# G-U-N/a-PyTorch-Tutorial-to-Class-Incremental-Learning

Measured on AMD Instinct MI355X. Metric: imgs/sec/node (CIFAR-100 B0-Inc10 ResNet-18 WA+KD step), higher is better.
Workload: dtype bf16; 1 GPU; model=resnet18, global_batch=128, input_size=32, kd=True, hip_graph=True, parallelism=dp1

## Files before the change

### cilfw/_hip_ops.py

```python

import ctypes
import os

import torch

_LIB_PATH = os.path.join(os.path.dirname(os.path.abspath(__file__)),
                         "_hip_lib.so")
if not os.path.exists(_LIB_PATH):
    raise ImportError(f"cilfw HIP library not built: {_LIB_PATH}")
_lib = ctypes.CDLL(_LIB_PATH)

_DEBUG = os.environ.get("CILFW_SYNC_DEBUG") == "1"

c_vp = ctypes.c_void_p
c_i = ctypes.c_int
c_l = ctypes.c_long
c_f = ctypes.c_float

_lib.cilfw_sync.restype = c_i
_lib.cilfw_error_string.restype = ctypes.c_char_p
_lib.cilfw_error_string.argtypes = [c_i]

_PROTOS = {
    "cilfw_conv2d_fwd": [c_vp] * 4 + [c_i] * 12 + [c_vp, c_vp],
    "cilfw_conv2d_bwd_data": [c_vp] * 4 + [c_i] * 12 + [c_vp] * 5 + [c_i, c_vp],
    "cilfw_conv2d_bwd_weight": [c_vp] * 4 + [c_i] * 13 + [c_vp],
    "cilfw_fill_mtable": [c_vp] + [c_i] * 4 + [c_vp],
    "cilfw_im2col_smallc": [c_vp] * 3 + [c_i] * 11 + [c_vp],
    "cilfw_bn_apply_only": [c_vp] * 7 + [c_l, c_i, c_i, c_vp],
    "cilfw_bn_fwd": [c_vp] * 11 + [c_i, c_l, c_i, c_f, c_f, c_i, c_i, c_vp],
    "cilfw_bn_bwd": [c_vp] * 11 + [c_vp, c_i] + [c_l, c_i, c_i, c_i, c_vp],
    "cilfw_add_relu_fwd": [c_vp] * 3 + [c_l, c_vp],
    "cilfw_add_relu_bwd": [c_vp] * 3 + [c_l, c_vp],
    "cilfw_downsample_a_fwd": [c_vp] * 2 + [c_i] * 4 + [c_vp],
    "cilfw_downsample_a_bwd": [c_vp] * 2 + [c_i] * 4 + [c_vp],
    "cilfw_gap_fwd": [c_vp] * 2 + [c_i] * 3 + [c_vp],
    "cilfw_gap_bwd": [c_vp] * 2 + [c_i] * 3 + [c_vp],
    "cilfw_stride_gather": [c_vp] * 2 + [c_i] * 7 + [c_vp],
    "cilfw_stride_scatter": [c_vp] * 2 + [c_i] * 7 + [c_vp],
    "cilfw_maxpool_fwd": [c_vp] * 3 + [c_i] * 9 + [c_vp],
    "cilfw_maxpool_bwd": [c_vp] * 3 + [c_i] * 9 + [c_vp],
    "cilfw_linear_fwd": [c_vp] * 5 + [c_i] * 4 + [c_vp],
    "cilfw_linear_dx": [c_vp] * 4 + [c_i] * 4 + [c_vp],
    "cilfw_linear_dw": [c_vp] * 5 + [c_i] * 4 + [c_vp],
    "cilfw_ce_fwd": [c_vp] * 5 + [c_i, c_i, c_f, c_vp],
    "cilfw_ce_bwd": [c_vp] * 4 + [c_i, c_i, c_f, c_vp],
    "cilfw_kd_fwd": [c_vp] * 6 + [c_i, c_i, c_f, c_vp],
    "cilfw_kd_bwd": [c_vp] * 4 + [c_i, c_i, c_f, c_vp],
    "cilfw_wa_loss_fwd": [c_vp] * 8 + [c_i] * 3 + [c_f] * 3 + [c_vp],
    "cilfw_wa_loss_bwd": [c_vp] * 6 + [c_i] * 3 + [c_f] * 3 + [c_vp],
    "cilfw_sgd_step": [c_vp] * 4 + [c_l, c_vp, c_f, c_f, c_vp],
    "cilfw_topk_correct": [c_vp] * 3 + [c_i] * 3 + [c_vp],
    "cilfw_herding_select": [c_vp] * 3 + [c_i] * 3 + [c_vp],
    "cilfw_herding_select_batch": [c_vp] * 6 + [c_i] * 3 + [c_vp],
    "cilfw_crop_resize": [c_vp] * 7 + [c_i] * 7 + [c_vp],
    "cilfw_crop_resize_ragged": [c_vp] * 9 + [c_i] * 5 + [c_vp],
    "cilfw_nme_prototypes": [c_vp] * 3 + [c_i] * 2 + [c_vp],
    "cilfw_nme_topk": [c_vp] * 6 + [c_i] * 4 + [c_vp],
    "cilfw_pod_pool": [c_vp] * 2 + [c_i] * 4 + [c_vp],
    "cilfw_pod_dist": [c_vp] * 5 + [c_i] * 2 + [c_vp],
    "cilfw_pod_bwd": [c_vp] * 4 + [c_i] * 4 + [c_vp],
    "cilfw_rownorm_fwd": [c_vp] * 4 + [c_i] * 3 + [c_vp],
    "cilfw_rownorm_bwd": [c_vp] * 6 + [c_i] * 3 + [c_vp],
    "cilfw_cos_sum": [c_vp] * 2 + [c_i, c_f, c_vp],
    "cilfw_flat_dist": [c_vp] * 5 + [c_i] * 2 + [c_vp],
    "cilfw_flat_bwd": [c_vp] * 3 + [c_i] * 2 + [c_vp],
    "cilfw_mrank_fwd": [c_vp] * 9 + [c_i] * 4 + [c_f, c_vp],
    "cilfw_mrank_bwd": [c_vp] * 6 + [c_i] * 4 + [c_vp],
}
for _name, _args in _PROTOS.items():
    _fn = getattr(_lib, _name)
    _fn.argtypes = _args
    _fn.restype = None

_lib.cilfw_conv2d_bwd_data.restype = c_i
for _name in ("cilfw_pod_pool", "cilfw_pod_dist", "cilfw_pod_bwd",
              "cilfw_rownorm_fwd", "cilfw_rownorm_bwd", "cilfw_cos_sum",
              "cilfw_flat_dist", "cilfw_flat_bwd", "cilfw_mrank_fwd",
              "cilfw_mrank_bwd"):
    getattr(_lib, _name).restype = c_i

for _name, _n in [("cilfw_linear_ksplit", 3),
                  ("cilfw_conv2d_fwd_ksplit", 7),
                  ("cilfw_conv2d_bwd_data_ksplit", 7),
                  ("cilfw_conv2d_bwd_data_can_fuse_bn", 8),
                  ("cilfw_conv2d_bwd_data_bn_gy", 3),
                  ("cilfw_conv2d_fwd_bn_gy", 3),
                  ("cilfw_bnbwd_fuse_enabled", 0),
                  ("cilfw_conv2d_bwd_weight_nslices", 7),
                  ("cilfw_conv2d_fwd_route", 8),
                  ("cilfw_conv2d_bwd_data_route", 9),
                  ("cilfw_conv2d_bwd_weight_route", 8),
                  ("cilfw_pod_supported", 4),
                  ("cilfw_pod_pool_groups", 2),
                  ("cilfw_cosine_supported", 3),
                  ("cilfw_mrank_supported", 4)]:
    _fn = getattr(_lib, _name)
    _fn.argtypes = [c_i] * _n
    _fn.restype = c_i
_lib.cilfw_bn_sums_gy.argtypes = [c_l]
_lib.cilfw_bn_sums_gy.restype = c_i

_FWD_ROUTES = ("v1_bk32", "v1_bk64", "v2_bn64", "v2_bn128")
_BWD_DATA_ROUTES = ("s2_fused", "v2", "v1_bk32", "v1_bk64")
_BWD_WEIGHT_ROUTES = ("v2", "v1_fast", "v1_generic")


def _stream():
    return c_vp(torch.cuda.current_stream().cuda_stream)


def _ptr(t):
    return c_vp(0 if t is None else t.data_ptr())


def _check(name):
    if _DEBUG:
        e = _lib.cilfw_sync()
        if e != 0:
            raise RuntimeError(
                f"HIP error after {name}: "
                f"{_lib.cilfw_error_string(e).decode()}")


def _bf16(t, name):
    assert t.dtype == torch.bfloat16, \
        f"{name}: GPU compute path is bf16 (got {t.dtype}); run with " \
        f"--dtype bf16 or set CILFW_FORCE_TORCH=1 for debugging"
    assert t.is_contiguous(), f"{name}: needs contiguous tensor"
    return t



def _out_hw(H, W_, R, S, stride, pad):
    return ((H + 2 * pad - R) // stride + 1,
            (W_ + 2 * pad - S) // stride + 1)


def _crs_pad(C, R, S):
    return (C * R * S + 15) // 16 * 16


def _slab_ws(nslabs, numel, device, always=False):
    if nslabs > 1 or always:
        return torch.empty(nslabs * numel, dtype=torch.float32, device=device)
    return None


def _stem_as_1x1(x, R, S, stride, pad, Ho, Wo):
    N, H, W_, C = x.shape
    M, CRSpad = N * Ho * Wo, _crs_pad(C, R, S)
    mt = _mtable(N, Ho, Wo, stride, x.device)
    col = torch.zeros(M, 1, 1, CRSpad, dtype=torch.bfloat16, device=x.device)
    _lib.cilfw_im2col_smallc(_ptr(x), _ptr(mt), _ptr(col), c_i(N), c_i(H),
                             c_i(W_), c_i(C), c_i(R), c_i(S), c_i(stride),
                             c_i(pad), c_i(Ho), c_i(Wo), c_i(CRSpad),
                             _stream())
    _check("im2col_smallc")
    return col


def conv2d_fwd_route(N, H, W_, C, K, R, S, stride, pad):
    Ho, Wo = _out_hw(H, W_, R, S, stride, pad)
    ks = _lib.cilfw_conv2d_fwd_ksplit(N, C, K, R, S, Ho, Wo)
    return _FWD_ROUTES[_lib.cilfw_conv2d_fwd_route(N, C, K, R, S, Ho, Wo,
                                                   ks)], ks


def conv2d_bwd_data_route(N, H, W_, C, K, R, S, stride):
    if R == 1 and S == 1 and stride > 1:
        H, W_, stride = (H - 1) // stride + 1, (W_ - 1) // stride + 1, 1
    ks = _lib.cilfw_conv2d_bwd_data_ksplit(N, H, W_, C, K, R, S)
    return _BWD_DATA_ROUTES[_lib.cilfw_conv2d_bwd_data_route(
        N, H, W_, C, K, R, S, stride, ks)], ks


def bnbwd_fuse_enabled():
    return bool(_lib.cilfw_bnbwd_fuse_enabled())


def _stem_im2col_dw(C, K, R, S):
    use_im2col = (os.environ.get("CILFW_STEM_IM2COL") == "1"
                  or (R * S >= 25
                      and os.environ.get("CILFW_STEM_IM2COL") != "0"))
    return C < 16 and R * S > 1 and K % 16 == 0 and use_im2col


def conv2d_bwd_weight_route(N, C, K, R, S, Ho, Wo, accum=False):
    if _stem_im2col_dw(C, K, R, S):
        N, C, R, S, Ho, Wo = N * Ho * Wo, _crs_pad(C, R, S), 1, 1, 1, 1
        accum = False
    ns = _lib.cilfw_conv2d_bwd_weight_nslices(N, C, K, R, S, Ho, Wo)
    return _BWD_WEIGHT_ROUTES[_lib.cilfw_conv2d_bwd_weight_route(
        N, C, K, R, S, Ho, Wo, 1 if accum else 0)], ns


def conv2d_fwd(x, w, stride, pad, want_bn_parts=False):
    _bf16(x, "conv2d_fwd.x")
    _bf16(w, "conv2d_fwd.w")
    N, H, W_, C = x.shape
    R, S, Cw, K = w.shape
    assert Cw == C
    assert K % 8 == 0, "conv kernels vector-stage over output channels (K%8==0)"
    Ho, Wo = _out_hw(H, W_, R, S, stride, pad)
    if C < 16 and R * S > 1 and K % 16 == 0 \
            and os.environ.get("CILFW_STEM_IM2COL") == "1":
        col = _stem_as_1x1(x, R, S, stride, pad, Ho, Wo)
        wpad = torch.zeros(1, 1, col.shape[-1], K, dtype=torch.bfloat16,
                           device=x.device)
        wpad[0, 0, :C * R * S] = w.reshape(C * R * S, K)
        y, _ = conv2d_fwd(col, wpad, 1, 0)
        return y.view(N, Ho, Wo, K), None
    y = torch.empty(N, Ho, Wo, K, dtype=torch.bfloat16, device=x.device)
    ks = _lib.cilfw_conv2d_fwd_ksplit(N, C, K, R, S, Ho, Wo)
    ws = _slab_ws(ks, y.numel(), x.device)
    parts = None
    if want_bn_parts and ks == 1 \
            and _FWD_ROUTES[_lib.cilfw_conv2d_fwd_route(
                N, C, K, R, S, Ho, Wo, ks)].startswith("v2_") \
            and os.environ.get("CILFW_CONV_BN_FUSE", "1") != "0":
        parts = torch.empty(_lib.cilfw_conv2d_fwd_bn_gy(N, Ho, Wo), 2, K,
                            dtype=torch.float32, device=x.device)
    _lib.cilfw_conv2d_fwd(_ptr(x), _ptr(w), _ptr(y), _ptr(ws), c_i(N),
                          c_i(H), c_i(W_), c_i(C), c_i(K), c_i(R), c_i(S),
                          c_i(stride), c_i(pad), c_i(Ho), c_i(Wo), c_i(ks),
                          _ptr(parts), _stream())
    _check("conv2d_fwd")
    return y, parts


def conv2d_bwd_data(dy, w, stride, pad, H, W_, bn_meta=None):
    _bf16(dy, "conv2d_bwd_data.dy")
    N, Ho, Wo, K = dy.shape
    R, S, C, Kw = w.shape
    assert Kw == K
    if R == 1 and S == 1 and stride > 1:
        dxs = conv2d_bwd_data(dy, w, 1, 0, Ho, Wo)
        dx = torch.empty(N, H, W_, C, dtype=torch.bfloat16, device=dy.device)
        _lib.cilfw_stride_scatter(_ptr(dxs), _ptr(dx), c_i(N), c_i(H),
                                  c_i(W_), c_i(C), c_i(stride), c_i(Ho),
                                  c_i(Wo), _stream())
        _check("stride_scatter")
        return (dx, None) if bn_meta is not None else dx
    dx = torch.empty(N, H, W_, C, dtype=torch.bfloat16, device=dy.device)
    ks = _lib.cilfw_conv2d_bwd_data_ksplit(N, H, W_, C, K, R, S)
    ws = _slab_ws(ks, dx.numel(), dy.device)
    parts = None
    bn_y = bn_x = bn_mean = bn_invstd = None
    bn_relu = False
    if (bn_meta is not None
            and _lib.cilfw_conv2d_bwd_data_can_fuse_bn(
                N, H, W_, C, K, R, S, stride)):
        bn_y, bn_x, bn_mean, bn_invstd, bn_relu = bn_meta
        parts = torch.empty(_lib.cilfw_conv2d_bwd_data_bn_gy(N, H, W_), 2, C,
                            dtype=torch.float32, device=dy.device)
    fused = _lib.cilfw_conv2d_bwd_data(
        _ptr(dy), _ptr(w), _ptr(dx), _ptr(ws), c_i(N), c_i(H), c_i(W_),
        c_i(C), c_i(K), c_i(R), c_i(S), c_i(stride), c_i(pad), c_i(Ho),
        c_i(Wo), c_i(ks), _ptr(bn_y), _ptr(bn_x), _ptr(bn_mean),
        _ptr(bn_invstd), _ptr(parts), c_i(1 if bn_relu else 0), _stream())
    if not fused:
        parts = None
    _check("conv2d_bwd_data")
    if bn_meta is not None:
        return dx, parts
    return dx


_mtable_cache = {}


def _mtable(N, Ho, Wo, stride, device):
    key = (N, Ho, Wo, stride, device)
    mt = _mtable_cache.get(key)
    if mt is None:
        assert N < 4096 and Ho * stride < 1024 and Wo * stride < 1024, \
            "mtable packing limits exceeded"
        M = N * Ho * Wo
        mt = torch.empty(M, dtype=torch.int32, device=device)
        _lib.cilfw_fill_mtable(_ptr(mt), c_i(M), c_i(Ho * Wo), c_i(Wo),
                               c_i(stride), _stream())
        _mtable_cache[key] = mt
    return mt


def conv2d_bwd_weight(dy, x, stride, pad, R, S, out=None, accum=False):
    _bf16(dy, "conv2d_bwd_weight.dy")
    _bf16(x, "conv2d_bwd_weight.x")
    N, H, W_, C = x.shape
    _, Ho, Wo, K = dy.shape
    if _stem_im2col_dw(C, K, R, S):
        col = _stem_as_1x1(x, R, S, stride, pad, Ho, Wo)
        dwp = conv2d_bwd_weight(dy.view(-1, 1, 1, K), col, 1, 0, 1, 1)
        dw = dwp.view(-1, K)[:C * R * S].reshape(R, S, C, K)
        if out is None:
            return dw
        (out.add_(dw) if accum else out.copy_(dw))
        return out
    if R == 1 and S == 1 and stride > 1:
        xg = torch.empty(N, Ho, Wo, C, dtype=torch.bfloat16, device=x.device)
        _lib.cilfw_stride_gather(_ptr(x), _ptr(xg), c_i(N), c_i(H), c_i(W_),
                                 c_i(C), c_i(stride), c_i(Ho), c_i(Wo),
                                 _stream())
        _check("stride_gather")
        return conv2d_bwd_weight(dy, xg, 1, 0, R, S, out=out, accum=accum)
    if out is None:
        dw = torch.empty(R, S, C, K, dtype=torch.float32, device=dy.device)
        accum = False
    else:
        assert out.is_contiguous() and out.dtype == torch.float32 \
            and out.shape == (R, S, C, K)
        dw = out
    ns = _lib.cilfw_conv2d_bwd_weight_nslices(N, C, K, R, S, Ho, Wo)
    ws = _slab_ws(ns, dw.numel(), dy.device, always=True)
    _lib.cilfw_conv2d_bwd_weight(_ptr(dy), _ptr(x), _ptr(dw),
                                 _ptr(ws), c_i(N), c_i(H), c_i(W_), c_i(C),
                                 c_i(K), c_i(R), c_i(S), c_i(stride),
                                 c_i(pad), c_i(Ho), c_i(Wo), c_i(ns),
                                 c_i(1 if accum else 0), _stream())
    _check("conv2d_bwd_weight")
    return dw



def bn_fwd(x, gamma, beta, running_mean, running_var, momentum, eps, training,
# ... 768 lines not shown
```

### cilfw/csrc/conv.hip

```cpp

#include "common.h"

#define BM 128
#define BN 64
#define NTHREADS 256

struct ConvGeom {
  int N, H, W, C, K, R, S, stride, pad, pad2, Ho, Wo;
  unsigned long long m_howo, m_wo;
  unsigned long long m_ck, m_s;
};

static inline unsigned long long magic40(int d) {
  return d > 0 ? ((1ULL << 40) / (unsigned)d + 1) : 0;
}

DEV unsigned mdiv40(unsigned n, unsigned long long m) {
  return (unsigned)(((unsigned long long)n * m) >> 40);
}

__global__ __launch_bounds__(NTHREADS)
void reduce_slabs_bf16_kernel(const float* __restrict__ ws,
                              bf16_t* __restrict__ out, int ns, long len) {
  long i0 = ((long)blockIdx.x * NTHREADS + threadIdx.x) * 4;
// ... 1278 lines not shown
      bool bok = m_ok & (ko0 + wv * 16 + lh * 8 + 8 <= g.K);
      const bf16_t* srcB = bok
          ? &dy[(long)mcl * g.K + ko0 + wv * 16 + lh * 8]
          : zpage;
      __builtin_amdgcn_global_load_lds(
          (const __attribute__((address_space(1))) unsigned int*)srcB,
          (__attribute__((address_space(3))) unsigned int*)
              &base[W2_IMG + wv * (WBK * 16) + i * 32 * 16], 16, 0, 0);
    }
  };

  const int fh = lane & 15, fq = lane >> 4;
  const unsigned lds0 = (unsigned)(uintptr_t)&lds[0];
  const unsigned tr_e = (unsigned)((fq * 8 + ((lane >> 2) & 3)) * 16
                                   + (lane & 3) * 4);

  const int nk = cdiv_i(me - ms, WBK);
  if (nk > 0) stage(0, ms);
  asm volatile("s_waitcnt vmcnt(0)" ::: "memory");
  __builtin_amdgcn_s_barrier();
  for (int kt = 0; kt < nk; ++kt) {
    int cur = kt & 1;
    if (kt + 1 < nk) stage(cur ^ 1, ms + (kt + 1) * WBK);
    const unsigned abase = lds0 + 2u * (cur * 2 * W2_IMG);
    const unsigned bbase = abase + 2u * W2_IMG;
    typedef __attribute__((ext_vector_type(4))) short s4_t;
#pragma unroll
    for (int kh = 0; kh < 2; ++kh) {
      const unsigned khe = 2u * (tr_e + kh * 32 * 16);
      bf16x8 afr[2], bfr[2];
#pragma unroll
      for (int mr = 0; mr < 2; ++mr) {
        unsigned a = abase + 2u * ((wr * 2 + mr) * (WBK * 16)) + khe;
        s4_t lo, hi;
        asm volatile("ds_read_b64_tr_b16 %0, %2\n\t"
                     "ds_read_b64_tr_b16 %1, %2 offset:128\n\t"
                     : "=&v"(lo), "=&v"(hi) : "v"(a));
        afr[mr] = __builtin_shufflevector(lo, hi, 0, 1, 2, 3, 4, 5, 6, 7);
      }
#pragma unroll
      for (int nr = 0; nr < 2; ++nr) {
        unsigned a = bbase + 2u * ((wc * 2 + nr) * (WBK * 16)) + khe;
        s4_t lo, hi;
        asm volatile("ds_read_b64_tr_b16 %0, %2\n\t"
                     "ds_read_b64_tr_b16 %1, %2 offset:128\n\t"
                     : "=&v"(lo), "=&v"(hi) : "v"(a));
        bfr[nr] = __builtin_shufflevector(lo, hi, 0, 1, 2, 3, 4, 5, 6, 7);
      }
      if (kh == 0) {
        asm volatile("s_waitcnt lgkmcnt(0)" ::: "memory");
        __builtin_amdgcn_sched_barrier(0);
        __builtin_amdgcn_s_setprio(1);
      } else {
        asm volatile("s_waitcnt lgkmcnt(0)" ::: "memory");
        __builtin_amdgcn_sched_barrier(0);
      }
#pragma unroll
      for (int mr = 0; mr < 2; ++mr)
#pragma unroll
        for (int nr = 0; nr < 2; ++nr)
          acc[mr][nr] = __builtin_amdgcn_mfma_f32_16x16x32_bf16(
              afr[mr], bfr[nr], acc[mr][nr], 0, 0, 0);
    }
    __builtin_amdgcn_s_setprio(0);
    asm volatile("s_waitcnt vmcnt(0)" ::: "memory");
    __builtin_amdgcn_s_barrier();
  }

  const long slab = (long)blockIdx.z * CRS * g.K;
#pragma unroll
  for (int mr = 0; mr < 2; ++mr)
#pragma unroll
    for (int nr = 0; nr < 2; ++nr)
#pragma unroll
      for (int r = 0; r < 4; ++r) {
        int row = rs0 + wr * 32 + mr * 16 + fq * 4 + r;
        int col = ko0 + wc * 32 + nr * 16 + fh;
        if (row < CRS && col < g.K)
          ws[slab + (long)row * g.K + col] = acc[mr][nr][r];
      }
}


#include <stdio.h>

#define KNOB_NEVER (1 << 30)

static int bk64_min_crs() {
  static const int v = env_int("CILFW_CONV_BK64_MIN", 512);
  return v > 0 ? v : KNOB_NEVER;
}

static int bk64_max_blocks() {
  static const int v = env_int("CILFW_CONV_BK64_MAXBLOCKS", 768);
  return v;
}

static int ksplit_target() {
  static const int v = env_int("CILFW_CONV_KSPLIT_TARGET", 512);
  return v;
}

static int dw_target() {
  static const int v = env_int("CILFW_CONV_DW_TARGET", 1024);
  return v;
}

static int conv_v2_enabled() {
  static const int v = env_int("CILFW_CONV_V2", 1);
  return v;
}

static int conv_v2_bwd_minm() {
  static const int v = env_int("CILFW_CONV_V2_BWD_MINM", 150000);
  return v == 0 ? KNOB_NEVER : v;
}

static int fwd_bm256_min_m() {
  static const int v = env_int("CILFW_CONV_BM256_MIN", 0);
  return v > 0 ? v : KNOB_NEVER;
}

static int v2_bn128_enabled() {
  static const int v = env_int("CILFW_CONV_V2_BN128", 1);
  return v;
}

static int v2_bn128_min3x3() {
  static const int v = env_int("CILFW_CONV_V2_BN128_MIN3X3", -1);
  return v >= 0 ? v : KNOB_NEVER;
}

static int s2_fused_enabled() {
  static const int v = !env_set("CILFW_NO_S2_FUSED");
  return v;
}

static int bnbwd_fuse_enabled() {
  static const int v = env_int("CILFW_BNBWD_FUSE", 0);
  return v;
}

static int pick_ksplit(int nblocks, int nk) {
  int ks = 1;
  while (ks < 8 && nblocks * ks < ksplit_target() && nk / (ks * 2) >= 4)
    ks *= 2;
  return ks;
}

static dim3 reduce_slabs_grid(long len) {
  return dim3((unsigned)((len + NTHREADS * 4 - 1) / (NTHREADS * 4)));
}

static void launch_reduce_slabs_bf16(const void* ws, void* out, int ksplit,
                                     long len, void* stream) {
  if (ksplit <= 1) return;
  hipLaunchKernelGGL(reduce_slabs_bf16_kernel, reduce_slabs_grid(len),
                     dim3(NTHREADS), 0, (hipStream_t)stream,
                     (const float*)ws, (bf16_t*)out, ksplit, len);
}

static void launch_reduce_slabs_f32(const void* ws, void* out, int nslices,
                                    long len, int accum, void* stream) {
  hipLaunchKernelGGL(reduce_slabs_f32_kernel, reduce_slabs_grid(len),
                     dim3(NTHREADS), 0, (hipStream_t)stream,
                     (const float*)ws, (float*)out, nslices, len, accum);
}

typedef void (*FwdV1Kernel)(const bf16_t*, const bf16_t*, bf16_t*, float*,
                            ConvGeom, int, int, int, int);
static const FwdV1Kernel kFwdV1[3][2] = {
    {conv2d_fwd_kernel<32, 128, BN, false>,
     conv2d_fwd_kernel<32, 128, BN, true>},
    {conv2d_fwd_kernel<64, 128, BN, false>,
     conv2d_fwd_kernel<64, 128, BN, true>},
    {conv2d_fwd_kernel<32, 256, BN, false>,
     conv2d_fwd_kernel<32, 256, BN, true>}};

typedef void (*BwdDataKernel)(const bf16_t*, const bf16_t*, bf16_t*, float*,
                              ConvGeom, int, int, int, int, const bf16_t*,
                              const bf16_t*, const float*, const float*,
                              float*, int);
static const BwdDataKernel kBwdData[2][2][2] = {
    {{conv2d_bwd_data_kernel<32, false, false>,
      conv2d_bwd_data_kernel<32, false, true>},
     {conv2d_bwd_data_kernel<32, true, false>,
      conv2d_bwd_data_kernel<32, true, true>}},
    {{conv2d_bwd_data_kernel<64, false, false>,
      conv2d_bwd_data_kernel<64, false, true>},
     {conv2d_bwd_data_kernel<64, true, false>,
      conv2d_bwd_data_kernel<64, true, true>}}};

extern "C" {

static void* zpage_ptr() {
  static void* p = nullptr;
  if (p == nullptr) {
    hipStreamCaptureStatus st = hipStreamCaptureStatusNone;
    (void)hipStreamIsCapturing(nullptr, &st);
    if (st != hipStreamCaptureStatusNone) return nullptr;
    void* q = nullptr;
    if (hipMalloc(&q, 65536) != hipSuccess) return nullptr;
    (void)hipMemset(q, 0, 65536);
    p = q;
  }
  return p;
}

enum { FWD_V1_BK32 = 0, FWD_V1_BK64 = 1, FWD_V2_BN64 = 2, FWD_V2_BN128 = 3 };
enum { BWDD_S2_FUSED = 0, BWDD_V2 = 1, BWDD_V1_BK32 = 2, BWDD_V1_BK64 = 3 };
enum { BWDW_V2 = 0, BWDW_V1_FAST = 1, BWDW_V1_GENERIC = 2 };

static int fwd_bm(int M) { return (M >= fwd_bm256_min_m()) ? 256 : BM; }

static int fwd_v2_eligible(int C) { return C % 8 == 0 && conv_v2_enabled(); }

static int fwd_route(int M, int C, int K, int R, int S, int ksplit,
                     int have_zp) {
  int CRS = C * R * S;
  int bm = fwd_bm(M);
  if (have_zp && fwd_v2_eligible(C) && bm == BM) {
    int shape_ok = (R == 1 && S == 1) || M >= v2_bn128_min3x3();
// ... 61 lines not shown
}

static int bwd_data_route(int N, int H, int W, int C, int K, int R, int S,
                          int stride, int ksplit, int have_zp) {
  int H2max = (H + 1) >> 1, W2max = (W + 1) >> 1;
  int Mc = N * H2max * W2max;
  if (stride == 2 && (R > 1 || S > 1) && K % 16 == 0 &&
      cdiv(Mc, BM) * cdiv(C, BN) >= 128 && s2_fused_enabled())
    return BWDD_S2_FUSED;
  int M = N * H * W;
  if (have_zp && bwd_data_v2_eligible(M, K, stride)) return BWDD_V2;
  int use64 = (R * S * K >= bk64_min_crs()) &&
              (cdiv(M, BM) * cdiv(C, BN) * ksplit < bk64_max_blocks());
  return use64 ? BWDD_V1_BK64 : BWDD_V1_BK32;
}

int cilfw_conv2d_bwd_data_route(int N, int H, int W, int C, int K, int R,
                                int S, int stride, int ksplit) {
  return bwd_data_route(N, H, W, C, K, R, S, stride, ksplit, 1);
}

int cilfw_conv2d_bwd_data_ksplit(int N, int H, int W, int C, int K, int R,
                                 int S) {
  return pick_ksplit(cdiv(N * H * W, BM) * cdiv(C, BN), cdiv(R * S * K, 32));
}

int cilfw_conv2d_bwd_data_can_fuse_bn(int N, int H, int W, int C, int K,
                                      int R, int S, int stride) {
  if (!bnbwd_fuse_enabled() || stride != 1) return 0;
  int ks = cilfw_conv2d_bwd_data_ksplit(N, H, W, C, K, R, S);
  int route = bwd_data_route(N, H, W, C, K, R, S, stride, ks, 1);
  return (route == BWDD_V1_BK32 || route == BWDD_V1_BK64) && ks == 1;
}

int cilfw_conv2d_bwd_data_bn_gy(int N, int H, int W) {
  return cdiv(N * H * W, BM);
}

int cilfw_conv2d_bwd_data(const void* dy, const void* w, void* dx, void* ws,
                          int N, int H, int W, int C, int K, int R, int S,
                          int stride, int pad, int Ho, int Wo, int ksplit,
                          const void* bn_y, const void* bn_x,
                          const void* bn_mean, const void* bn_invstd,
                          void* bn_parts, int bn_relu, void* stream) {
  ConvGeom g{N, H, W, C, K, R, S, stride, pad, pad, Ho, Wo,
             0, 0, magic40(K), magic40(S)};
  int M = N * H * W;
  int RSK = R * S * K;
  void* zp = bwd_data_v2_eligible(M, K, stride) ? zpage_ptr() : nullptr;
  int route = bwd_data_route(N, H, W, C, K, R, S, stride, ksplit,
                             zp != nullptr);
  if (route == BWDD_S2_FUSED) {
    int Mc = N * ((H + 1) >> 1) * ((W + 1) >> 1);
    dim3 grid(cdiv(Mc, BM), cdiv(C, BN), 4);
    hipLaunchKernelGGL((conv2d_bwd_data_s2_kernel<32>), grid, dim3(NTHREADS),
                       0, (hipStream_t)stream, (const bf16_t*)dy,
                       (const bf16_t*)w, (bf16_t*)dx, g);
    return 0;
  }
  dim3 grid(cdiv(M, BM), cdiv(C, BN), ksplit);
  int bnp = 0;
  if (route == BWDD_V2) {
    hipLaunchKernelGGL(conv2d_bwd_data_v2_kernel, grid, dim3(NTHREADS), 0,
                       (hipStream_t)stream, (const bf16_t*)dy,
                       (const bf16_t*)w, (bf16_t*)dx, (float*)ws,
                       (const bf16_t*)zp, g, M, RSK, cdiv(RSK, V2BK), ksplit);
  } else {
    int bk64 = route == BWDD_V1_BK64;
    int fast = (K % 16 == 0) && stride <= 2;
    bnp = bn_parts != nullptr && ksplit == 1 && stride == 1 &&
          bnbwd_fuse_enabled();
    hipLaunchKernelGGL(kBwdData[bk64][fast][bnp], grid, dim3(NTHREADS), 0,
                       (hipStream_t)stream, (const bf16_t*)dy,
                       (const bf16_t*)w, (bf16_t*)dx, (float*)ws, g, M, RSK,
                       cdiv(RSK, bk64 ? 64 : 32), ksplit,
                       (const bf16_t*)bn_y, (const bf16_t*)bn_x,
                       (const float*)bn_mean, (const float*)bn_invstd,
                       (float*)bn_parts, bn_relu);
  }
  launch_reduce_slabs_bf16(ws, dx, ksplit, (long)M * C, stream);
  return bnp;
}

static int bwd_weight_v2_eligible(int C, int K, int accum) {
  return C % 8 == 0 && K % 8 == 0 && accum == 0 && conv_v2_enabled();
}

static int bwd_weight_route(int C, int K, int accum, int have_zp) {
  if (have_zp && bwd_weight_v2_eligible(C, K, accum)) return BWDW_V2;
  return (C % 8 == 0) ? BWDW_V1_FAST : BWDW_V1_GENERIC;
}

int cilfw_conv2d_bwd_weight_route(int N, int C, int K, int R, int S, int Ho,
                                  int Wo, int accum) {
  (void)N; (void)R; (void)S; (void)Ho; (void)Wo;
  return bwd_weight_route(C, K, accum, 1);
}

void cilfw_conv2d_bwd_weight(const void* dy, const void* x, void* dw,
                             void* ws, int N, int H, int W, int C, int K,
                             int R, int S, int stride, int pad, int Ho,
                             int Wo, int nslices, int accum, void* stream) {
  ConvGeom g{N, H, W, C, K, R, S, stride, pad, pad, Ho, Wo,
             magic40(Ho * Wo), magic40(Wo), magic40(C), magic40(S)};
  int M = N * Ho * Wo;
  if (M >= (1 << 22) || Ho * Wo >= (1 << 14)) {
    fprintf(stderr, "cilfw_conv2d_bwd_weight: magic-division range exceeded "
            "(M=%d HoWo=%d)\n", M, Ho * Wo);
    abort();
  }
  int CRS = C * R * S;
  int slice_len = cdiv(cdiv(M, nslices), WBK) * WBK;
  dim3 grid(cdiv(CRS, WBM), cdiv(K, BN), nslices);
  void* zp = bwd_weight_v2_eligible(C, K, accum) ? zpage_ptr() : nullptr;
  int route = bwd_weight_route(C, K, accum, zp != nullptr);
  if (route == BWDW_V2)
    hipLaunchKernelGGL(conv2d_bwd_weight_v2_kernel, grid, dim3(NTHREADS), 0,
                       (hipStream_t)stream, (const bf16_t*)dy,
                       (const bf16_t*)x, (float*)ws, (const bf16_t*)zp, g,
                       M, CRS, slice_len);
  else
    hipLaunchKernelGGL(route == BWDW_V1_FAST
                           ? conv2d_bwd_weight_kernel<true>
                           : conv2d_bwd_weight_kernel<false>,
                       grid, dim3(NTHREADS), 0, (hipStream_t)stream,
                       (const bf16_t*)dy, (const bf16_t*)x, (float*)ws, g, M,
                       CRS, slice_len);
  launch_reduce_slabs_f32(ws, dw, nslices, (long)CRS * K, accum, stream);
}

void cilfw_im2col_smallc(const void* x, const void* mt, void* col,
                         int N, int H, int W, int C, int R, int S,
                         int stride, int pad, int Ho, int Wo, int CRSpad,
                         void* stream) {
  ConvGeom g{N, H, W, C, 0, R, S, stride, pad, pad, Ho, Wo};
  int M = N * Ho * Wo;
  long total = (long)M * R * S;
  hipLaunchKernelGGL(im2col_smallc_kernel,
                     dim3((int)cdiv((long)total, (long)NTHREADS)),
                     dim3(NTHREADS), 0, (hipStream_t)stream,
                     (const bf16_t*)x, (const int*)mt, (bf16_t*)col, g, M,
                     CRSpad, total);
}

void cilfw_fill_mtable(void* mt, int M, int HoWo, int Wo, int stride,
                       void* stream) {
  hipLaunchKernelGGL(fill_mtable_kernel, dim3(cdiv(M, NTHREADS)),
                     dim3(NTHREADS), 0, (hipStream_t)stream, (int*)mt, M,
                     HoWo, Wo, stride);
}

int cilfw_conv2d_bwd_weight_nslices(int N, int C, int K, int R, int S,
                                    int Ho, int Wo) {
  int M = N * Ho * Wo;
  int CRS = C * R * S;
  int nblocks = cdiv(CRS, WBM) * cdiv(K, BN);
  int ns = cdiv(dw_target(), max(nblocks, 1));
  int max_ns = max(cdiv(M, WBK * 8), 1);
  if (ns > max_ns) ns = max_ns;
  if (ns < 1) ns = 1;
  if (ns > 64) ns = 64;
  return ns;
}

}
```

### cilfw/distributed/ddp.py

```python

import torch
import torch.distributed as dist


def _dist_active():
    return dist.is_available() and dist.is_initialized() and \
        dist.get_world_size() > 1


class DataParallelEngine:
    def __init__(self, model, bucket_mb=25.0, process_group=None):
        self.model = model
        self.group = process_group
        self.params = [p for p in model.parameters() if p.requires_grad]
        self.params = self.params[::-1]
        assert all(p.dtype == torch.float32 for p in self.params), \
            "cilfw keeps fp32 master params; compute casts are per-op"
        dev = self.params[0].device
        self.numel = sum(p.numel() for p in self.params)
        self.flat_params = torch.empty(self.numel, dtype=torch.float32, device=dev)
        self.flat_grads = torch.zeros(self.numel, dtype=torch.float32, device=dev)

        offset = 0
        self._offsets = []
        for p in self.params:
            n = p.numel()
            self.flat_params[offset:offset + n].copy_(p.data.reshape(-1))
            p.data = self.flat_params[offset:offset + n].view_as(p)
            p.grad = self.flat_grads[offset:offset + n].view_as(p)
            self._offsets.append(offset)
            offset += n

        bucket_elems = max(int(bucket_mb * 1024 * 1024 / 4), 1)
        self.buckets = []
        start, count, idxs = 0, 0, []
        for i, p in enumerate(self.params):
            idxs.append(i)
            count += p.numel()
            if count >= bucket_elems:
                self.buckets.append((start, start + count, tuple(idxs)))
                start += count
                count, idxs = 0, []
        if idxs:
            self.buckets.append((start, start + count, tuple(idxs)))
        self._param_bucket = {}
        for bi, (_, _, idxs) in enumerate(self.buckets):
            for i in idxs:
                self._param_bucket[i] = bi

        self._arrived = [0] * len(self.buckets)
        self._launched = [False] * len(self.buckets)
        self._works = []
        self._hooks = []
        self._hook_enabled = True
        for i, p in enumerate(self.params):
            self._hooks.append(p.register_post_accumulate_grad_hook(
                self._make_hook(i)))

        self._epoch = 0
        self._side_dirty = False
        for i, p in enumerate(self.params):
            p._cilfw_sink = (self, i)
            p._cilfw_sink_epoch = -1

        if _dist_active():
            dist.broadcast(self.flat_params, src=0, group=self.group)

        self.flat_bf16 = None
        if self.flat_params.is_cuda:
            self.flat_bf16 = self.flat_params.to(torch.bfloat16)
            for p, off in zip(self.params, self._offsets):
                p._cilfw_bf16 = self.flat_bf16[off:off + p.numel()].view_as(p)

    def _make_hook(self, i):
        bi = self._param_bucket[i]

        def hook(_p):
            if not self._hook_enabled:
                return
            self._arrived[bi] += 1
            if self._arrived[bi] == len(self.buckets[bi][2]):
                self._launch(bi)
        return hook

    def _launch(self, bi):
        if self._launched[bi] or not _dist_active():
            self._launched[bi] = True
            return
        self._join_side_stream()
        s, e, _ = self.buckets[bi]
        work = dist.all_reduce(self.flat_grads[s:e], op=dist.ReduceOp.SUM,
                               group=self.group, async_op=True)
        self._works.append(work)
        self._launched[bi] = True


    def sink_acquire(self, i):
        p = self.params[i]
        off = self._offsets[i]
        view = self.flat_grads[off:off + p.numel()]
        return view, p._cilfw_sink_epoch == self._epoch

    def sink_delivered(self, i, side_stream=False):
        p = self.params[i]
        p._cilfw_sink_epoch = self._epoch
        if side_stream:
            self._side_dirty = True
        if self._hook_enabled:
            bi = self._param_bucket[i]
            self._arrived[bi] += 1
            if self._arrived[bi] == len(self.buckets[bi][2]):
                self._launch(bi)

    def _join_side_stream(self):
        if self._side_dirty and self.flat_grads.is_cuda:
            from ..ops.functional import _wstream
            torch.cuda.current_stream().wait_stream(_wstream())
        self._side_dirty = False

    def zero_grad(self):
        self.flat_grads.zero_()
        self._arrived = [0] * len(self.buckets)
        self._launched = [False] * len(self.buckets)
        self._works = []
        self._epoch += 1

    def finalize(self):
        for bi in range(len(self.buckets)):
            if not self._launched[bi]:
                self._launch(bi)
        self._join_side_stream()
        for w in self._works:
            w.wait()
        self._works = []
        if _dist_active():
            self.flat_grads.mul_(1.0 / dist.get_world_size(group=self.group))

    def no_sync(self):
        engine = self

        class _NoSync:
            def __enter__(self):
                engine._hook_enabled = False

            def __exit__(self, *a):
                engine._hook_enabled = True
        return _NoSync()

    def detach(self):
        for h in self._hooks:
            h.remove()
        for p in self.params:
            p.data = p.data.clone()
            p.grad = None
            if hasattr(p, "_cilfw_bf16"):
                del p._cilfw_bf16
            if hasattr(p, "_cilfw_sink"):
                del p._cilfw_sink
                del p._cilfw_sink_epoch
```

### cilfw/ops/functional.py

```python

import torch
import torch.nn.functional as F

from ._backend import use_hip, ext, _load


_wgrad_stream = None


def _wstream():
    global _wgrad_stream
    if _wgrad_stream is None:
        _wgrad_stream = torch.cuda.Stream()
    return _wgrad_stream


def _to_nchw(x):
    return x.permute(0, 3, 1, 2).contiguous()


def _to_nhwc(x):
    return x.permute(0, 2, 3, 1).contiguous()




def _sink_on():
    import os
    return os.environ.get("CILFW_SINK_MODE", "join") != "off"


def _bnbwd_fuse_on():
    E = _load()
    if E is not None:
        return E.bnbwd_fuse_enabled()
    import os
    return os.environ.get("CILFW_BNBWD_FUSE", "0") == "1"


def _conv_bwd_data_with_bn(ctx, E, dy, wc, stride, padding, x):
    meta = getattr(ctx, "bnbwd_src", None)
    if meta is None or not _bnbwd_fuse_on():
        return E.conv2d_bwd_data(dy, wc, stride, padding,
                                 x.shape[1], x.shape[2])
    bn_x, bn_mean, bn_invstd, bn_relu = meta
    dx, parts = E.conv2d_bwd_data(
        dy, wc, stride, padding, x.shape[1], x.shape[2],
        bn_meta=(x, bn_x, bn_mean, bn_invstd, bn_relu))
    if parts is not None:
        dx._cilfw_bnbwd = (parts, bn_mean)
    return dx


class Conv2dNHWC(torch.autograd.Function):

    @staticmethod
    def forward(ctx, x, w, stride, padding, w_param=None):
        ctx.stride, ctx.padding = stride, padding
        if w_param is not None:
            w_param = w_param[0]
        wp = w_param if w_param is not None else w
        wc = getattr(wp, "_cilfw_bf16", None)
        if wc is None or wc.dtype != x.dtype:
            wc = w.to(x.dtype)
        ctx.save_for_backward(x, wc)
        ctx.w_dtype = w.dtype
        ctx.w_ref = wp
        ctx.sinked = w_param is not None
        ctx.bnbwd_src = getattr(x, "_cilfw_bnbwd_src", None)
        if use_hip(x):
            y, parts = ext().conv2d_fwd(x, wc, stride, padding,
                                        want_bn_parts=ctx.sinked)
            if parts is not None:
                y._cilfw_bn_parts = parts
            return y
        xf = _to_nchw(x).float()
        wf = w.permute(3, 2, 0, 1).contiguous().float()
        y = F.conv2d(xf, wf, stride=stride, padding=padding)
        return _to_nhwc(y).to(x.dtype)

    @staticmethod
    def backward(ctx, dy):
        x, wc = ctx.saved_tensors
        stride, padding = ctx.stride, ctx.padding
        dy = dy.contiguous()
        need_dx = ctx.needs_input_grad[0]
        sink = getattr(ctx.w_ref, "_cilfw_sink", None) if ctx.sinked else None
        if use_hip(dy):
            R, S = wc.shape[0], wc.shape[1]
            cur = torch.cuda.current_stream()
            ws = _wstream()
            ws.wait_stream(cur)
            if sink is not None:
                eng, pi = sink
                slot, accum = eng.sink_acquire(pi)
                out = slot.view(R, S, wc.shape[2], wc.shape[3])
                with torch.cuda.stream(ws):
                    ext().conv2d_bwd_weight(dy, x, stride, padding, R, S,
                                            out=out, accum=accum)
                dx = _conv_bwd_data_with_bn(ctx, ext(), dy, wc, stride, padding, x) \
                    if need_dx else None
                cur.wait_stream(ws)
                eng.sink_delivered(pi)
                return dx, None, None, None, None
            with torch.cuda.stream(ws):
                dw = ext().conv2d_bwd_weight(dy, x, stride, padding, R, S)
            dx = _conv_bwd_data_with_bn(ctx, ext(), dy, wc, stride, padding, x) \
                if need_dx else None
            cur.wait_stream(ws)
            dw.record_stream(cur)
            return dx, dw.to(ctx.w_dtype), None, None, None
        xf = _to_nchw(x).float()
        wf = wc.permute(3, 2, 0, 1).contiguous().float()
        dyf = _to_nchw(dy).float()
        dx = None
        if need_dx:
            dxf = torch.nn.grad.conv2d_input(xf.shape, wf, dyf, stride=stride,
                                             padding=padding)
            dx = _to_nhwc(dxf).to(x.dtype)
        dwf = torch.nn.grad.conv2d_weight(xf, wf.shape, dyf, stride=stride,
                                          padding=padding)
        dw = dwf.permute(2, 3, 1, 0).contiguous().to(ctx.w_dtype)
        if sink is not None:
            eng, pi = sink
            slot, accum = eng.sink_acquire(pi)
            out = slot.view_as(dw)
            (out.add_(dw) if accum else out.copy_(dw))
# ... 630 lines not shown
```

### cilfw/optim.py

```python

import math

import torch

from .ops._backend import use_hip, ext


class FlatSGD:
    def __init__(self, engine, lr, momentum=0.9, weight_decay=5e-4):
        self.engine = engine
        self._lr_dev = (torch.full((1,), float(lr), dtype=torch.float32,
                                   device=engine.flat_params.device)
                        if engine.flat_params.is_cuda else None)
        self._lr = float(lr)
        self.base_lr = lr
        self.momentum = momentum
        self.weight_decay = weight_decay
        self.momentum_buf = torch.zeros_like(engine.flat_grads)

    @property
    def lr(self):
        return self._lr

    @lr.setter
    def lr(self, v):
        self._lr = float(v)
        if self._lr_dev is not None:
            self._lr_dev.fill_(float(v))

    @torch.no_grad()
    def step(self):
        p, g, m = (self.engine.flat_params, self.engine.flat_grads,
                   self.momentum_buf)
        mirror = getattr(self.engine, "flat_bf16", None)
        if use_hip(p):
            ext().sgd_step(p, g, m, self._lr_dev, self.momentum,
                           self.weight_decay, mirror)
            return
        if self.weight_decay != 0:
            g = g.add(p, alpha=self.weight_decay)
        m.mul_(self.momentum).add_(g)
        p.add_(m, alpha=-self.lr)
        if mirror is not None:
            mirror.copy_(p)

    def zero_grad(self):
        self.engine.zero_grad()

    def state_dict(self):
        return {"lr": self.lr, "base_lr": self.base_lr,
                "momentum": self.momentum, "weight_decay": self.weight_decay,
                "momentum_buf": self.momentum_buf}

    def load_state_dict(self, sd):
        self.lr = sd["lr"]
        self.base_lr = sd["base_lr"]
        self.momentum = sd["momentum"]
        self.weight_decay = sd["weight_decay"]
        self.momentum_buf.copy_(sd["momentum_buf"])


class CosineLR:

    def __init__(self, optimizer, t_max, eta_min=0.0):
        self.opt = optimizer
        self.t_max = t_max
        self.eta_min = eta_min
        self.epoch = 0

    def step(self):
        self.epoch += 1
        self.opt.lr = self.eta_min + (self.opt.base_lr - self.eta_min) * \
            (1 + math.cos(math.pi * min(self.epoch, self.t_max) / self.t_max)) / 2

    def state_dict(self):
        return {"epoch": self.epoch, "t_max": self.t_max, "eta_min": self.eta_min}

    def load_state_dict(self, sd):
        self.epoch = sd["epoch"]
        self.t_max = sd["t_max"]
        self.eta_min = sd["eta_min"]
```

Measured before the change: 41860 imgs/s.

## Compute conv backward-data as forward conv over pre-flipped transposed weights

```diff
diff --git a/cilfw/_hip_ops.py b/cilfw/_hip_ops.py
--- a/cilfw/_hip_ops.py
+++ b/cilfw/_hip_ops.py
@@ -25,6 +25,8 @@
     "cilfw_conv2d_fwd": [c_vp] * 4 + [c_i] * 12 + [c_vp, c_vp],
     "cilfw_conv2d_bwd_data": [c_vp] * 4 + [c_i] * 12 + [c_vp] * 5 + [c_i, c_vp],
     "cilfw_conv2d_bwd_weight": [c_vp] * 4 + [c_i] * 13 + [c_vp],
+    "cilfw_conv2d_bwd_data_flipped": [c_vp] * 4 + [c_i] * 11 + [c_vp],
+    "cilfw_conv_wflip": [c_vp] * 3 + [c_i, c_i, c_vp],
     "cilfw_fill_mtable": [c_vp] + [c_i] * 4 + [c_vp],
     "cilfw_im2col_smallc": [c_vp] * 3 + [c_i] * 11 + [c_vp],
     "cilfw_bn_apply_only": [c_vp] * 7 + [c_l, c_i, c_i, c_vp],
@@ -85,6 +87,9 @@
                   ("cilfw_conv2d_bwd_data_ksplit", 7),
                   ("cilfw_conv2d_bwd_data_can_fuse_bn", 8),
                   ("cilfw_conv2d_bwd_data_bn_gy", 3),
+                  ("cilfw_conv2d_bwd_flip_enabled", 0),
+                  ("cilfw_conv2d_bwd_flip_eligible", 9),
+                  ("cilfw_conv2d_bwd_flip_ksplit", 7),
                   ("cilfw_conv2d_fwd_bn_gy", 3),
                   ("cilfw_bnbwd_fuse_enabled", 0),
                   ("cilfw_conv2d_bwd_weight_nslices", 7),
@@ -229,18 +234,99 @@
     return y, parts
 
 
-def conv2d_bwd_data(dy, w, stride, pad, H, W_, bn_meta=None):
+def conv2d_bwd_flip_enabled():
+    return bool(_lib.cilfw_conv2d_bwd_flip_enabled())
+
+
+def conv2d_bwd_flip_eligible(N, H, W_, C, K, R, S, stride, pad):
+    return bool(_lib.cilfw_conv2d_bwd_flip_eligible(N, H, W_, C, K, R, S,
+                                                    stride, pad))
+
+
+def conv2d_bwd_flip_route(N, H, W_, C, K, R, S, pad):
+    Ho, Wo = _out_hw(H, W_, R, S, 1, pad)
+    ks = _lib.cilfw_conv2d_bwd_flip_ksplit(N, H, W_, C, K, R, S)
+    return _FWD_ROUTES[_lib.cilfw_conv2d_fwd_route(N, K, C, R, S, H, W_,
+                                                   ks)], ks
+
+
+def conv2d_bwd_data_flipped(dy, wT, pad, H, W_, out=None):
+    _bf16(dy, "conv2d_bwd_data_flipped.dy")
+    _bf16(wT, "conv2d_bwd_data_flipped.wT")
+    N, Ho, Wo, K = dy.shape
+    R, S, Kw, C = wT.shape
+    assert Kw == K and R == S and 0 <= pad <= R - 1
+    assert C % 8 == 0 and K % 8 == 0
+    assert (Ho, Wo) == _out_hw(H, W_, R, S, 1, pad)
+    if out is None:
+        out = torch.empty(N, H, W_, C, dtype=torch.bfloat16, device=dy.device)
+    assert out.shape == (N, H, W_, C) and out.is_contiguous() \
+        and out.dtype == torch.bfloat16
+    ks = _lib.cilfw_conv2d_bwd_flip_ksplit(N, H, W_, C, K, R, S)
+    ws = _slab_ws(ks, out.numel(), dy.device)
+    _lib.cilfw_conv2d_bwd_data_flipped(
+        _ptr(dy), _ptr(wT), _ptr(out), _ptr(ws), c_i(N), c_i(H), c_i(W_),
+        c_i(C), c_i(K), c_i(R), c_i(S), c_i(pad), c_i(Ho), c_i(Wo), c_i(ks),
+        _stream())
+    _check("conv2d_bwd_data_flipped")
+    return out
+
+
+_WFLIP_ALIGN = 8
+
+
+def wflip_layout(shapes):
+    offs, total = [], 0
+    for R, S, C, K in shapes:
+        offs.append(total)
+        total += (R * S * C * K + _WFLIP_ALIGN - 1) // _WFLIP_ALIGN \
+            * _WFLIP_ALIGN
+    return offs, total
+
+
+def wflip_table(entries, src_numel, dst_numel, device):
+    rows, tiles = [], 0
+    for so, do, R, S, C, K in entries:
+        n = R * S * C * K
+        assert C % 8 == 0 and K % 8 == 0, "conv_wflip moves 8-element rows"
+        assert do % _WFLIP_ALIGN == 0, "conv_wflip stores 16-byte rows"
+        assert 0 <= so and so + n <= src_numel
+        assert 0 <= do and do + n <= dst_numel
+        rows.append([so, do, R, S, C, K, tiles])
+        tiles += R * S * ((C + 63) // 64) * ((K + 63) // 64)
+    assert tiles < 2 ** 31
+    tab = torch.tensor(rows, dtype=torch.int64).reshape(-1, 7).to(device)
+    return tab, tiles
+
+
+def conv_wflip(src, dst, tab, ntiles):
+    _bf16(src, "conv_wflip.src")
+    _bf16(dst, "conv_wflip.dst")
+    assert tab.dtype == torch.int64 and tab.is_contiguous() \
+        and tab.dim() == 2 and tab.shape[1] == 7
+    assert dst.data_ptr() % 16 == 0
+    _lib.cilfw_conv_wflip(_ptr(src), _ptr(dst), _ptr(tab),
+                          c_i(tab.shape[0]), c_i(ntiles), _stream())
+    _check("conv_wflip")
+
+
+def conv2d_bwd_data(dy, w, stride, pad, H, W_, bn_meta=None, w_flipped=None):
     _bf16(dy, "conv2d_bwd_data.dy")
     N, Ho, Wo, K = dy.shape
     R, S, C, Kw = w.shape
     assert Kw == K
     if R == 1 and S == 1 and stride > 1:
-        dxs = conv2d_bwd_data(dy, w, 1, 0, Ho, Wo)
+        dxs = conv2d_bwd_data(dy, w, 1, 0, Ho, Wo, w_flipped=w_flipped)
         dx = torch.empty(N, H, W_, C, dtype=torch.bfloat16, device=dy.device)
         _lib.cilfw_stride_scatter(_ptr(dxs), _ptr(dx), c_i(N), c_i(H),
                                   c_i(W_), c_i(C), c_i(stride), c_i(Ho),
                                   c_i(Wo), _stream())
         _check("stride_scatter")
+        return (dx, None) if bn_meta is not None else dx
+    if w_flipped is not None and conv2d_bwd_flip_eligible(
+            N, H, W_, C, K, R, S, stride, pad):
+        assert w_flipped.shape == (R, S, K, C)
+        dx = conv2d_bwd_data_flipped(dy, w_flipped, pad, H, W_)
         return (dx, None) if bn_meta is not None else dx
     dx = torch.empty(N, H, W_, C, dtype=torch.bfloat16, device=dy.device)
     ks = _lib.cilfw_conv2d_bwd_data_ksplit(N, H, W_, C, K, R, S)
diff --git a/cilfw/csrc/conv.hip b/cilfw/csrc/conv.hip
--- a/cilfw/csrc/conv.hip
+++ b/cilfw/csrc/conv.hip
@@ -1384,6 +1384,67 @@
 }
 
 
+#define WF_T 64
+#define WF_LP (WF_T + 8)
+#define WF_COLS 7
+
+__global__ __launch_bounds__(NTHREADS)
+void conv_wflip_kernel(const bf16_t* __restrict__ src,
+                       bf16_t* __restrict__ dst,
+                       const long long* __restrict__ tab, int nconv) {
+  __shared__ __align__(16) bf16_t tile[WF_T * WF_LP];
+  const int b = blockIdx.x;
+  int lo = 0, hi = nconv - 1;
+  while (lo < hi) {
+    int mid = (lo + hi + 1) >> 1;
+    if (tab[mid * WF_COLS + 6] <= b) lo = mid; else hi = mid - 1;
+  }
+  const long long* d = tab + lo * WF_COLS;
+  const int R = (int)d[2], S = (int)d[3], C = (int)d[4], K = (int)d[5];
+  const int tk = cdiv_i(K, WF_T), tc = cdiv_i(C, WF_T);
+  int lt = b - (int)d[6];
+  const int kt = lt % tk;
+  lt /= tk;
+  const int ct = lt % tc;
+  const int rs = lt / tc;
+  if (rs >= R * S) return;
+  const int r = rs / S, s = rs - r * S;
+  const bf16_t* sp = src + d[0] + (long)rs * C * K;
+  bf16_t* op = dst + d[1] + (long)((R - 1 - r) * S + (S - 1 - s)) * K * C;
+  const int c0 = ct * WF_T, k0 = kt * WF_T;
+  const int t = threadIdx.x, row = t >> 3, ch = (t & 7) * 8;
+  const bool al16 = (((uintptr_t)(src + d[0])) & 15) == 0;
+#pragma unroll
+  for (int h = 0; h < 2; ++h) {
+    const int c = row + h * 32;
+    int4 v{0, 0, 0, 0};
+    if (c0 + c < C && k0 + ch < K) {
+      const bf16_t* p = sp + (long)(c0 + c) * K + k0 + ch;
+      if (al16) {
+        v = *(const int4*)p;
+      } else {
+        __align__(16) bf16_t tmp[8];
+#pragma unroll
+        for (int j = 0; j < 8; ++j) tmp[j] = p[j];
+        v = *(int4*)tmp;
+      }
+    }
+    *(int4*)&tile[c * WF_LP + ch] = v;
+  }
+  __syncthreads();
+#pragma unroll
+  for (int h = 0; h < 2; ++h) {
+    const int k = row + h * 32;
+    if (k0 + k < K && c0 + ch < C) {
+      __align__(16) bf16_t tmp[8];
+#pragma unroll
+      for (int j = 0; j < 8; ++j) tmp[j] = tile[(ch + j) * WF_LP + k];
+      *(int4*)(op + (long)(k0 + k) * C + c0 + ch) = *(int4*)tmp;
+    }
+  }
+}
+
+
 #include <stdio.h>
 
 #define KNOB_NEVER (1 << 30)
@@ -1440,6 +1501,11 @@
 
 static int bnbwd_fuse_enabled() {
   static const int v = env_int("CILFW_BNBWD_FUSE", 0);
+  return v;
+}
+
+static int bwd_flip_enabled() {
+  static const int v = env_int("CILFW_CONV_BWD_FLIP", 1);
   return v;
 }
 
@@ -1667,6 +1733,45 @@
   return bnp;
 }
 
+static int bwd_flip_gate(int M, int C, int K, int R) {
+  if (R == 1 && C > K && M >= 32768) return 0;
+  return 1;
+}
+
+int cilfw_conv2d_bwd_flip_enabled() {
+  if (!bwd_flip_enabled() || !conv_v2_enabled()) return 0;
+  return !bnbwd_fuse_enabled();
+}
+
+int cilfw_conv2d_bwd_flip_eligible(int N, int H, int W, int C, int K, int R,
+                                   int S, int stride, int pad) {
+  if (!cilfw_conv2d_bwd_flip_enabled()) return 0;
+  if (stride != 1 || R != S || pad < 0 || pad > R - 1) return 0;
+  if (C % 8 != 0 || K % 8 != 0) return 0;
+  return bwd_flip_gate(N * H * W, C, K, R);
+}
+
+int cilfw_conv2d_bwd_flip_ksplit(int N, int H, int W, int C, int K, int R,
+                                 int S) {
+  return cilfw_conv2d_fwd_ksplit(N, K, C, R, S, H, W);
+}
+
+void cilfw_conv2d_bwd_data_flipped(const void* dy, const void* wT, void* dx,
+                                   void* ws, int N, int H, int W, int C,
+                                   int K, int R, int S, int pad, int Ho,
+                                   int Wo, int ksplit, void* stream) {
+  cilfw_conv2d_fwd(dy, wT, dx, ws, N, Ho, Wo, K, C, R, S, 1, R - 1 - pad, H,
+                   W, ksplit, nullptr, stream);
+}
+
+void cilfw_conv_wflip(const void* src, void* dst, const void* tab, int nconv,
+                      int ntiles, void* stream) {
+  if (nconv <= 0 || ntiles <= 0) return;
+  hipLaunchKernelGGL(conv_wflip_kernel, dim3(ntiles), dim3(NTHREADS), 0,
+                     (hipStream_t)stream, (const bf16_t*)src, (bf16_t*)dst,
+                     (const long long*)tab, nconv);
+}
+
 static int bwd_weight_v2_eligible(int C, int K, int accum) {
   return C % 8 == 0 && K % 8 == 0 && accum == 0 && conv_v2_enabled();
 }
diff --git a/cilfw/distributed/ddp.py b/cilfw/distributed/ddp.py
--- a/cilfw/distributed/ddp.py
+++ b/cilfw/distributed/ddp.py
@@ -71,6 +71,54 @@
             self.flat_bf16 = self.flat_params.to(torch.bfloat16)
             for p, off in zip(self.params, self._offsets):
                 p._cilfw_bf16 = self.flat_bf16[off:off + p.numel()].view_as(p)
+        self.flat_bf16_t = None
+        self._wflip = None
+        self._build_flipped()
+
+    def _build_flipped(self):
+        from ..ops._backend import have_ext
+        if self.flat_bf16 is None or not have_ext():
+            return
+        from ..ops._backend import ext
+        E = ext()
+        if not E.conv2d_bwd_flip_enabled():
+            return
+        convs = {}
+        for m in self.model.modules():
+            w = getattr(m, "weight", None)
+            if (w is not None and w.dim() == 4 and hasattr(m, "kernel_size")
+                    and hasattr(m, "stride")):
+                convs[id(w)] = m
+        picked = []
+        for p, off in zip(self.params, self._offsets):
+            m = convs.get(id(p))
+            if m is None:
+                continue
+            R, S, C, K = p.shape
+            if (R == S and C % 8 == 0 and K % 8 == 0
+                    and (m.stride == 1 or R == 1)):
+                picked.append((p, off))
+        if not picked:
+            return
+        offs, total = E.wflip_layout([tuple(p.shape) for p, _ in picked])
+        self.flat_bf16_t = torch.zeros(total, dtype=torch.bfloat16,
+                                       device=self.flat_bf16.device)
+        entries = []
+        for (p, off), doff in zip(picked, offs):
+            R, S, C, K = p.shape
+            entries.append((off, doff, R, S, C, K))
+            p._cilfw_bf16_t = self.flat_bf16_t[doff:doff + p.numel()].view(
+                R, S, K, C)
+        self._wflip = E.wflip_table(entries, self.flat_bf16.numel(), total,
+                                    self.flat_bf16.device)
+        self.refresh_flipped()
+
+    def refresh_flipped(self):
+        if self._wflip is None:
+            return
+        from ..ops._backend import ext
+        tab, ntiles = self._wflip
+        ext().conv_wflip(self.flat_bf16, self.flat_bf16_t, tab, ntiles)
 
     def _make_hook(self, i):
         bi = self._param_bucket[i]
@@ -155,6 +203,8 @@
             p.grad = None
             if hasattr(p, "_cilfw_bf16"):
                 del p._cilfw_bf16
+            if hasattr(p, "_cilfw_bf16_t"):
+                del p._cilfw_bf16_t
             if hasattr(p, "_cilfw_sink"):
                 del p._cilfw_sink
                 del p._cilfw_sink_epoch
diff --git a/cilfw/ops/functional.py b/cilfw/ops/functional.py
--- a/cilfw/ops/functional.py
+++ b/cilfw/ops/functional.py
@@ -38,11 +38,23 @@
     return os.environ.get("CILFW_BNBWD_FUSE", "0") == "1"
 
 
+def _flipped_mirror(ctx, wc):
+    if not ctx.sinked:
+        return None
+    mirror = getattr(ctx.w_ref, "_cilfw_bf16", None)
+    wT = getattr(ctx.w_ref, "_cilfw_bf16_t", None)
+    if (mirror is None or wT is None or wc.data_ptr() != mirror.data_ptr()
+            or wc.shape != mirror.shape or wc.dtype != mirror.dtype):
+        return None
+    return wT
+
+
 def _conv_bwd_data_with_bn(ctx, E, dy, wc, stride, padding, x):
     meta = getattr(ctx, "bnbwd_src", None)
     if meta is None or not _bnbwd_fuse_on():
         return E.conv2d_bwd_data(dy, wc, stride, padding,
-                                 x.shape[1], x.shape[2])
+                                 x.shape[1], x.shape[2],
+                                 w_flipped=_flipped_mirror(ctx, wc))
     bn_x, bn_mean, bn_invstd, bn_relu = meta
     dx, parts = E.conv2d_bwd_data(
         dy, wc, stride, padding, x.shape[1], x.shape[2],
diff --git a/cilfw/optim.py b/cilfw/optim.py
--- a/cilfw/optim.py
+++ b/cilfw/optim.py
@@ -36,6 +36,7 @@
         if use_hip(p):
             ext().sgd_step(p, g, m, self._lr_dev, self.momentum,
                            self.weight_decay, mirror)
+            self._refresh_flipped()
             return
         if self.weight_decay != 0:
             g = g.add(p, alpha=self.weight_decay)
@@ -43,6 +44,12 @@
         p.add_(m, alpha=-self.lr)
         if mirror is not None:
             mirror.copy_(p)
+            self._refresh_flipped()
+
+    def _refresh_flipped(self):
+        refresh = getattr(self.engine, "refresh_flipped", None)
+        if refresh is not None:
+            refresh()
 
     def zero_grad(self):
         self.engine.zero_grad()
```

New measurement: 42220 imgs/s (median of 6 runs). Within noise of the previous version (+0.9%).
